# scroll-tech/zkevm-circuits

Measured on AMD Instinct MI355X. Metric: SuperCircuit-shape proof-gen wall-clock (s) at k = 20, lower is better.
Workload: dtype u32x8 limbs (254-bit modular integer, Montgomery)

## Files before the change

### zkevm-circuits_amd/csrc/ntt.hip

```cpp
#include "ctx.hpp"
#include "ff29.hip.hpp"

namespace zk {

constexpr int NTT_MAX_DIGIT = 10;
constexpr int NTT_TILE = 4096;
constexpr int NTT_THREADS = 1024;
constexpr int NTT_LDS_BYTES_PER_ELT = 36;

struct Tw29;

constexpr int NTT_BATCH = 16;
struct NttIo { const Fr* src[NTT_BATCH]; Fr* dst[NTT_BATCH]; };

struct NttPass {
    int log_np;
    int log_m;
    const Tw29* tw;
    const Fr* out_tw = nullptr;
};

struct NttDomain {
    uint32_t log_n = 0;
    int npass = 0;
    NttPass pass[3];
    int h = 0;
    Fr* d_lo = nullptr;
    Fr* d_hi = nullptr;
    Fr* d_tw[3] = {nullptr, nullptr, nullptr};
    Tw29* d_tw29[3] = {nullptr, nullptr, nullptr};
    Fr* d_out_tw[2] = {nullptr, nullptr};
    Fr final_mul;
    bool fin_folded = false;
    ~NttDomain() {
        if (d_lo) (void)hipFree(d_lo);
        if (d_hi) (void)hipFree(d_hi);
        for (auto p : d_tw) if (p) (void)hipFree(p);
        for (auto p : d_tw29) if (p) (void)hipFree((void*)p);
        for (auto p : d_out_tw) if (p) (void)hipFree(p);
    }
};

__device__ __forceinline__ uint32_t bitrev(uint32_t x, int bits) { return bits ? (__brev(x) >> (32 - bits)) : 0u; }

__host__ __device__ __forceinline__ Fr to_rprime(Fr x) {
#pragma unroll
    for (int i = 0; i < 5; ++i) x = dbl(x);
    return x;
}

struct Lds29 {
    uint32_t* p;
    int stride;
    __device__ __forceinline__ Fr29 load(int idx) const {
        Fr29 r;
#pragma unroll
        for (int k = 0; k < 9; ++k) r.l[k] = p[k * stride + idx];
        return r;
    }
    __device__ __forceinline__ void store(int idx, const Fr29& v) const {
#pragma unroll
        for (int k = 0; k < 9; ++k) p[k * stride + idx] = v.l[k];
    }
};

__global__ void k_powers(Fr base, Fr mul, Fr* out, uint32_t count, int rprime) {
    uint32_t j = blockIdx.x * blockDim.x + threadIdx.x;
    if (j >= count) return;
    Fr r = mul, b = base;
    uint32_t e = j;
    while (e) {
        if (e & 1) r = r * b;
        b = sqr(b);
        e >>= 1;
    }
    stg(out + j, rprime ? to_rprime(r) : r);
}

__device__ __forceinline__ Fr two_level(const Fr* __restrict__ lo, const Fr* __restrict__ hi, int h, uint32_t e) {
    return ldg(lo + (e & ((1u << h) - 1))) * ldg(hi + (e >> h));
}
__device__ __forceinline__ Fr29 two_level29(const Fr* __restrict__ lo, const Fr* __restrict__ hi, int h, uint32_t e) {
    return mul29(unpack29<Fr29P>(ldg(lo + (e & ((1u << h) - 1)))), unpack29<Fr29P>(ldg(hi + (e >> h))));
}

__global__ void k_build_out_twiddles(Fr* __restrict__ out_tw, const Fr* __restrict__ lo, const Fr* __restrict__ hi, int h, int log_np, int log_m, int tw_shift, uint64_t n,
                                     Fr fin, int apply_fin) {
    const uint64_t g = (uint64_t)blockIdx.x * blockDim.x + threadIdx.x;
    if (g >= n) return;
    const uint64_t m = 1ull << log_m;
    const uint32_t jpp = (uint32_t)(g & (m - 1)), d = (uint32_t)(g >> log_m) & ((1u << log_np) - 1);
    Fr29 v = two_level29(lo, hi, h, (jpp * d) << tw_shift);
    if (apply_fin) v = mul29(v, unpack29<Fr29P>(fin));
    stg(out_tw + g, pack29_lt2p(v));
}

__device__ __forceinline__ void bfly29(Fr29& u, Fr29& x, const Fr29& w) {
    const Fr29 v = mul29(x, w);
    Fr29 a0 = add29(u, v), a1 = sub29k<4>(u, v);
    normalize29(a0);
    normalize29(a1);
    u = a0;
    x = a1;
}
struct Tw29 { uint4 q[3]; };
__device__ __forceinline__ Fr29 tw29(const Tw29* __restrict__ tw, uint32_t idx) {
    const uint4 a = tw[idx].q[0], b = tw[idx].q[1], c = tw[idx].q[2];
    return Fr29{{a.x, a.y, a.z, a.w, b.x, b.y, b.z, b.w, c.x}};
}
__global__ void k_split_twiddles(const Fr* __restrict__ in, Tw29* __restrict__ out, uint32_t count) {
    const uint32_t i = blockIdx.x * blockDim.x + threadIdx.x;
    if (i >= count) return;
    const Fr29 v = unpack29<Fr29P>(ldg(in + i));
    out[i].q[0] = make_uint4(v.l[0], v.l[1], v.l[2], v.l[3]);
    out[i].q[1] = make_uint4(v.l[4], v.l[5], v.l[6], v.l[7]);
    out[i].q[2] = make_uint4(v.l[8], 0u, 0u, 0u);
}
__device__ __forceinline__ void bfly29_lazy(Fr29& u, Fr29& x, const Fr29& w) {
    const Fr29 v = mul29(x, w);
    const Fr29 a0 = add29(u, v), a1 = sub29k<2>(u, v);
    u = a0;
    x = a1;
}
template <int R>
__device__ __forceinline__ void dit_step(Fr29 (&e)[4], const Tw29* __restrict__ tw, int log_np, int s, int j) {
    const Fr29 w0 = tw29(tw, (uint32_t)j << (log_np - 1 - s));
    bfly29_lazy(e[0], e[1], w0);
    if (R == 2) {
        bfly29_lazy(e[2], e[3], w0);
        bfly29_lazy(e[0], e[2], tw29(tw, (uint32_t)j << (log_np - 2 - s)));
        bfly29_lazy(e[1], e[3], tw29(tw, (uint32_t)(j + (1 << s)) << (log_np - 2 - s)));
        normalize29(e[2]);
        normalize29(e[3]);
    }
    normalize29(e[0]);
    normalize29(e[1]);
}
__device__ __forceinline__ void bfly29_one(Fr29& u, Fr29& x) {
    Fr29 a0 = add29(u, x), a1 = sub29k<4>(u, x);
    normalize29(a0);
    normalize29(a1);
    u = a0;
    x = a1;
}
template <int R>
__device__ __forceinline__ void dit_first_step(Fr29 (&e)[4], const Tw29* __restrict__ tw, int log_np) {
    bfly29_one(e[0], e[1]);
    if (R == 2) {
        bfly29_one(e[2], e[3]);
        bfly29_one(e[0], e[2]);
        bfly29(e[1], e[3], tw29(tw, 1u << (log_np - 2)));
    }
}

__global__ void __launch_bounds__(NTT_THREADS)
k_ntt_pass(NttIo io, const Tw29* __restrict__ tw, const Fr* __restrict__ lo,
           const Fr* __restrict__ hi, int h, int log_np, int log_t, int log_m, int tw_shift, const Fr* __restrict__ pre,
           const Fr* __restrict__ out_tw, uint32_t ncols, int xcd_cols) {
    extern __shared__ __attribute__((aligned(16))) uint32_t smem[];
    uint32_t tile_id, col;
    if (xcd_cols) { const uint32_t slot = blockIdx.x >> 3; col = slot % ncols; tile_id = (slot / ncols) * 8u + (blockIdx.x & 7u); }
    else { col = blockIdx.x % ncols; tile_id = blockIdx.x / ncols; }
    const Fr* __restrict__ src = io.src[col];
    Fr* __restrict__ dst = io.dst[col];
    const int tile = 1 << (log_np + log_t);
    Lds29 L{smem, tile};
    const int T = 1 << log_t;
    const uint64_t m = 1ull << log_m;
    const uint32_t tiles_per_hi = (uint32_t)(m >> log_t);
    const uint32_t hi_idx = tile_id / tiles_per_hi, blk = tile_id % tiles_per_hi;
    const uint64_t base = ((uint64_t)hi_idx << (log_np + log_m)) + ((uint64_t)blk << log_t);

    for (int s = 0; s < log_np;) {
        const int r = ((log_np - s) & 1) ? 1 : 2;
        const bool first = s == 0, last = s + r == log_np;
        const int hgt = 1 << s, items = tile >> r;
        for (int it = threadIdx.x; it < items; it += blockDim.x) {
            const int c = it & (T - 1), b = it >> log_t;
            const int j = b & (hgt - 1);
            const int lo_d = ((b >> s) << (s + r)) | j;
            Fr29 e[4];
#pragma unroll
            for (int k = 0; k < 4; ++k) {
                if (k >= (1 << r)) break;
                const int dl = lo_d + k * hgt;
                if (first) {
                    const uint64_t gi = base + (uint64_t)bitrev(dl, log_np) * m + c;
                    e[k] = unpack29<Fr29P>(ldg(src + gi));
                    if (pre) e[k] = mul29(e[k], unpack29<Fr29P>(ldg(pre + gi)));
                } else {
                    e[k] = L.load((dl << log_t) | c);
                }
            }
            if (first) { if (r == 2) dit_first_step<2>(e, tw, log_np); else dit_first_step<1>(e, tw, log_np); }
            else if (r == 2) dit_step<2>(e, tw, log_np, s, j);
            else dit_step<1>(e, tw, log_np, s, j);
#pragma unroll
            for (int k = 0; k < 4; ++k) {
                if (k >= (1 << r)) break;
                const int dl = lo_d + k * hgt;
                if (last) {
                    const uint32_t jpp = (blk << log_t) + c;
                    const uint64_t go = base + (uint64_t)dl * m + c;
                    const Fr29 v = mul29(e[k], out_tw ? unpack29<Fr29P>(ldg(out_tw + go)) : two_level29(lo, hi, h, (jpp * (uint32_t)dl) << tw_shift));
                    stg(dst + go, pack29_raw(v));
                } else {
                    L.store((dl << log_t) | c, e[k]);
                }
            }
        }
        s += r;
        if (s < log_np) __syncthreads();
    }
}

static bool ntt_xcd_remap() { static const bool on = getenv("ZK_NTT_XCD") && atoi(getenv("ZK_NTT_XCD")) == 1; return on; }
__host__ __device__ __forceinline__ int ntt_row_pad(int log_np) { return log_np >= 8 ? 8 : 0; }
__global__ void __launch_bounds__(NTT_THREADS)
k_ntt_last(NttIo io, const Tw29* __restrict__ tw, int log_np, int log_t,
           int log_n1, int log_mid, Fr fin, const Fr* __restrict__ pre, int fin_folded, int xcd_remap) {
    extern __shared__ __attribute__((aligned(16))) uint32_t smem[];
    const Fr* __restrict__ src = io.src[blockIdx.y];
    Fr* __restrict__ dst = io.dst[blockIdx.y];
    const int tile = 1 << (log_np + log_t);
    const int T = 1 << log_t;
    const int row = (1 << log_np) + ntt_row_pad(log_np);
    Lds29 L{smem, T * row};
    uint32_t bx = blockIdx.x;
    if (xcd_remap) bx = (bx & 7u) * (gridDim.x >> 3) + (bx >> 3);
    const uint32_t mid = bx & ((1u << log_mid) - 1), blk = bx >> log_mid;
    const Fr29 fin29 = unpack29<Fr29P>(fin);

    for (int s = 0; s < log_np;) {
        const int r = ((log_np - s) & 1) ? 1 : 2;
        const bool first = s == 0, last = s + r == log_np;
        const int hgt = 1 << s, items = tile >> r;
        for (int it = threadIdx.x; it < items; it += blockDim.x) {
            int c, b;
            if (last) { c = it & (T - 1); b = it >> log_t; }
            else { b = it & ((1 << (log_np - r)) - 1); c = it >> (log_np - r); }
            const int j = b & (hgt - 1);
            const int lo_d = ((b >> s) << (s + r)) | j;
            const uint64_t i1 = ((uint64_t)blk << log_t) + c;
            Fr29 e[4];
#pragma unroll
            for (int k = 0; k < 4; ++k) {
                if (k >= (1 << r)) break;
                const int dl = lo_d + k * hgt;
                if (first) {
                    const uint64_t gi = (((i1 << log_mid) + mid) << log_np) + bitrev(dl, log_np);
                    e[k] = unpack29<Fr29P>(ldg(src + gi));
                    if (pre) e[k] = mul29(e[k], unpack29<Fr29P>(ldg(pre + gi)));
                } else {
                    e[k] = L.load(c * row + dl);
                }
            }
            if (first) { if (r == 2) dit_first_step<2>(e, tw, log_np); else dit_first_step<1>(e, tw, log_np); }
            else if (r == 2) dit_step<2>(e, tw, log_np, s, j);
            else dit_step<1>(e, tw, log_np, s, j);
#pragma unroll
            for (int k = 0; k < 4; ++k) {
                if (k >= (1 << r)) break;
                const int dl = lo_d + k * hgt;
                if (last) {
                    const uint64_t o = i1 + (((uint64_t)mid + ((uint64_t)dl << log_mid)) << log_n1);
                    stg(dst + o, fin_folded ? reduce_lazy29(e[k]) : pack29_lt2p(mul29(e[k], fin29)));
                } else {
                    L.store(c * row + dl, e[k]);
                }
            }
        }
        s += r;
        if (s < log_np) __syncthreads();
    }
}


template <int LOG_NP, int S, bool HAS_PRE>
__device__ __forceinline__ void ntt_pass_steps(const Lds29& L, const Fr* __restrict__ src, Fr* __restrict__ dst, const Tw29* __restrict__ tw,
                                               const Fr* __restrict__ pre, const Fr* __restrict__ out_tw, const int log_t, const uint64_t m, const uint64_t base) {
    constexpr int R = ((LOG_NP - S) & 1) ? 1 : 2, NE = 1 << R, hgt = 1 << S;
    constexpr bool FIRST = S == 0, LAST = S + R == LOG_NP;
    const int T = 1 << log_t, items = (1 << (LOG_NP + log_t)) >> R;
    for (int it = threadIdx.x; it < items; it += blockDim.x) {
        const int c = it & (T - 1), b = it >> log_t;
        const int j = b & (hgt - 1);
        const int lo_d = ((b >> S) << (S + R)) | j;
        Fr otw[NE];
        if (LAST) {
#pragma unroll
            for (int k = 0; k < NE; ++k) otw[k] = ldg(out_tw + base + (uint64_t)(lo_d + k * hgt) * m + c);
        }
        Fr29 e[4];
        if (FIRST) {
            Fr raw[NE], praw[NE];
#pragma unroll
            for (int k = 0; k < NE; ++k) {
                const uint64_t gi = base + (uint64_t)bitrev(lo_d + k * hgt, LOG_NP) * m + c;
                raw[k] = ldg(src + gi);
                if (HAS_PRE) praw[k] = ldg(pre + gi);
            }
#pragma unroll
            for (int k = 0; k < NE; ++k) {
                e[k] = unpack29<Fr29P>(raw[k]);
                if (HAS_PRE) e[k] = mul29(e[k], unpack29<Fr29P>(praw[k]));
            }
            dit_first_step<R>(e, tw, LOG_NP);
        } else {
#pragma unroll
            for (int k = 0; k < NE; ++k) e[k] = L.load(((lo_d + k * hgt) << log_t) | c);
            dit_step<R>(e, tw, LOG_NP, S, j);
        }
#pragma unroll
        for (int k = 0; k < NE; ++k) {
            const int dl = lo_d + k * hgt;
            if (LAST) stg(dst + base + (uint64_t)dl * m + c, pack29_raw(mul29(e[k], unpack29<Fr29P>(otw[k]))));
            else L.store((dl << log_t) | c, e[k]);
        }
    }
    if constexpr (!LAST) {
        __syncthreads();
        ntt_pass_steps<LOG_NP, S + R, HAS_PRE>(L, src, dst, tw, pre, out_tw, log_t, m, base);
    }
}
template <int LOG_NP, bool HAS_PRE>
__global__ void __launch_bounds__(NTT_THREADS)
k_ntt_pass_f(NttIo io, const Tw29* __restrict__ tw, int log_t, int log_m, const Fr* __restrict__ pre, const Fr* __restrict__ out_tw, uint32_t ncols, int xcd_cols, int log_grp) {
    extern __shared__ __attribute__((aligned(16))) uint32_t smem[];
    uint32_t tile_id, col;
    if (xcd_cols) {
        const uint32_t slot = blockIdx.x >> 3, sub = slot & ((1u << log_grp) - 1u), s2 = slot >> log_grp;
        col = s2 % ncols;
        tile_id = ((((s2 / ncols) << 3) + (blockIdx.x & 7u)) << log_grp) + sub;
    } else { col = blockIdx.x % ncols; tile_id = blockIdx.x / ncols; }
    Lds29 L{smem, 1 << (LOG_NP + log_t)};
    const uint64_t m = 1ull << log_m;
    const uint32_t tiles_per_hi = (uint32_t)(m >> log_t);
    const uint32_t hi_idx = tile_id / tiles_per_hi, blk = tile_id % tiles_per_hi;
    const uint64_t base = ((uint64_t)hi_idx << (LOG_NP + log_m)) + ((uint64_t)blk << log_t);
    ntt_pass_steps<LOG_NP, 0, HAS_PRE>(L, io.src[col], io.dst[col], tw, pre, out_tw, log_t, m, base);
}

template <int LOG_NP, int S>
__device__ __forceinline__ void ntt_last_steps(const Lds29& L, const Fr* __restrict__ src, Fr* __restrict__ dst, const Tw29* __restrict__ tw,
                                               const int log_t, const int row, const uint32_t blk, const uint32_t mid, const int log_mid, const int log_n1) {
    constexpr int R = ((LOG_NP - S) & 1) ? 1 : 2, NE = 1 << R, hgt = 1 << S;
    constexpr bool FIRST = S == 0, LAST = S + R == LOG_NP;
    const int T = 1 << log_t, items = (1 << (LOG_NP + log_t)) >> R;
    for (int it = threadIdx.x; it < items; it += blockDim.x) {
        int c, b;
        if (LAST) { c = it & (T - 1); b = it >> log_t; }
        else { b = it & ((1 << (LOG_NP - R)) - 1); c = it >> (LOG_NP - R); }
        const int j = b & (hgt - 1);
        const int lo_d = ((b >> S) << (S + R)) | j;
        const uint64_t i1 = ((uint64_t)blk << log_t) + c;
        Fr29 e[4];
        if (FIRST) {
            Fr raw[NE];
#pragma unroll
            for (int k = 0; k < NE; ++k) raw[k] = ldg(src + ((((i1 << log_mid) + mid) << LOG_NP) + bitrev(lo_d + k * hgt, LOG_NP)));
#pragma unroll
            for (int k = 0; k < NE; ++k) e[k] = unpack29<Fr29P>(raw[k]);
            dit_first_step<R>(e, tw, LOG_NP);
        } else {
#pragma unroll
            for (int k = 0; k < NE; ++k) e[k] = L.load(c * row + lo_d + k * hgt);
            dit_step<R>(e, tw, LOG_NP, S, j);
        }
#pragma unroll
        for (int k = 0; k < NE; ++k) {
            const int dl = lo_d + k * hgt;
            if (LAST) stg(dst + (i1 + (((uint64_t)mid + ((uint64_t)dl << log_mid)) << log_n1)), reduce_lazy29(e[k]));
            else L.store(c * row + dl, e[k]);
        }
    }
    if constexpr (!LAST) {
        __syncthreads();
        ntt_last_steps<LOG_NP, S + R>(L, src, dst, tw, log_t, row, blk, mid, log_mid, log_n1);
    }
}
template <int LOG_NP>
__global__ void __launch_bounds__(NTT_THREADS)
k_ntt_last_f(NttIo io, const Tw29* __restrict__ tw, int log_t, int log_n1, int log_mid, int xcd_remap) {
    extern __shared__ __attribute__((aligned(16))) uint32_t smem[];
    const int row = (1 << LOG_NP) + ntt_row_pad(LOG_NP);
    Lds29 L{smem, (1 << log_t) * row};
    uint32_t bx = blockIdx.x;
    if (xcd_remap) bx = (bx & 7u) * (gridDim.x >> 3) + (bx >> 3);
    const uint32_t mid = bx & ((1u << log_mid) - 1), blk = bx >> log_mid;
    ntt_last_steps<LOG_NP, 0>(L, io.src[blockIdx.y], io.dst[blockIdx.y], tw, log_t, row, blk, mid, log_mid, log_n1);
}

__global__ void k_scale(Fr* a, Fr s, uint64_t n) {
    uint64_t i = (uint64_t)blockIdx.x * blockDim.x + threadIdx.x;
    if (i < n) stg(a + i, ldg(a + i) * s);
}
int fr_scale_run(zk_ctx* ctx, Fr* d_a, const Fr& s, uint64_t n) {
    if (!n) return ZK_OK;
    hipLaunchKernelGGL(k_scale, dim3((unsigned)((n + 255) / 256)), dim3(256), 0, ctx->stream, d_a, s, n);
    ZK_CHECK_LAUNCH(ctx);
    return ZK_OK;
}

__global__ void k_distribute_powers(const Fr* src, Fr* dst, const Fr* __restrict__ lo, const Fr* __restrict__ hi, int h, uint64_t n) {
    uint64_t i = (uint64_t)blockIdx.x * blockDim.x + threadIdx.x;
    if (i >= n) return;
    stg(dst + i, ldg(src + i) * two_level(lo, hi, h, (uint32_t)i));
}

static int build_powers(zk_ctx* ctx, const Fr& base, const Fr& mul, Fr* d_out, uint32_t count, int rprime) {
    hipLaunchKernelGGL(k_powers, dim3((count + 255) / 256), dim3(256), 0, ctx->stream, base, mul, d_out, count, rprime);
    ZK_CHECK_LAUNCH(ctx);
    return ZK_OK;
}

static uint64_t domain_key(uint32_t log_n, const Fr& omega, const Fr* scale) {
    uint64_t hsh = 1469598103934665603ull;
    auto mix = [&](uint32_t v) { hsh = (hsh ^ v) * 1099511628211ull; };
    mix(log_n);
    for (int i = 0; i < 8; ++i) mix(omega.l[i]);
    if (scale) for (int i = 0; i < 8; ++i) mix(scale->l[i] ^ 0x9e3779b9u);
    return hsh;
}

static int get_domain(zk_ctx* ctx, uint32_t log_n, const Fr& omega, const Fr* scale, std::shared_ptr<NttDomain>* out) {
    const uint64_t key = domain_key(log_n, omega, scale);
    auto it = ctx->domains.find(key);
    if (it != ctx->domains.end()) { *out = it->second; return ZK_OK; }
    auto d = std::make_shared<NttDomain>();
    d->log_n = log_n;
    d->final_mul = to_rprime(scale ? *scale : Fr::one());
    const int P = log_n <= NTT_MAX_DIGIT ? 1 : (log_n <= 2 * NTT_MAX_DIGIT ? 2 : 3);
    d->npass = P;
    int rem = (int)log_n;
    for (int p = 0; p < P; ++p) {
        int b = (rem + (P - p) - 1) / (P - p);
        d->pass[p].log_np = b;
        rem -= b;
        d->pass[p].log_m = rem;
    }
    if (P > 1) {
        d->h = (int)(log_n + 1) / 2;
        const uint32_t nlo = 1u << d->h, nhi = 1u << (log_n - d->h);
        ZK_HIP(ctx, hipMalloc(&d->d_lo, sizeof(Fr) * nlo));
        ZK_HIP(ctx, hipMalloc(&d->d_hi, sizeof(Fr) * nhi));
        int rc = build_powers(ctx, omega, Fr::one(), d->d_lo, nlo, 1);
        if (rc) return rc;
        Fr step = omega;
        for (int i = 0; i < d->h; ++i) step = sqr(step);
        rc = build_powers(ctx, step, Fr::one(), d->d_hi, nhi, 1);
        if (rc) return rc;
    }
    for (int p = 0; p < P; ++p) {
        const int b = d->pass[p].log_np;
        const uint32_t cnt = b ? (1u << (b - 1)) : 1u;
        ZK_HIP(ctx, hipMalloc(&d->d_tw[p], sizeof(Fr) * cnt));
        Fr w = omega;
        for (uint32_t i = 0; i < log_n - (uint32_t)b; ++i) w = sqr(w);
        int rc = build_powers(ctx, w, Fr::one(), d->d_tw[p], cnt, 1);
        if (rc) return rc;
        ZK_HIP(ctx, hipMalloc((void**)&d->d_tw29[p], sizeof(Tw29) * cnt));
        hipLaunchKernelGGL(k_split_twiddles, dim3((cnt + 255) / 256), dim3(256), 0, ctx->stream, (const Fr*)d->d_tw[p], d->d_tw29[p], cnt);
        ZK_CHECK_LAUNCH(ctx);
        d->pass[p].tw = d->d_tw29[p];
    }
    if (P > 1 && log_n <= 24) {
        const uint64_t n = 1ull << log_n;
        for (int p = 0; p + 1 < P; ++p) {
            if (hipMalloc(&d->d_out_tw[p], sizeof(Fr) * n) != hipSuccess) { (void)hipGetLastError(); d->d_out_tw[p] = nullptr; break; }
            const NttPass& ps = d->pass[p];
            hipLaunchKernelGGL(k_build_out_twiddles, dim3((unsigned)((n + 255) / 256)), dim3(256), 0, ctx->stream, d->d_out_tw[p], (const Fr*)d->d_lo, (const Fr*)d->d_hi, d->h,
                               ps.log_np, ps.log_m, (int)log_n - ps.log_np - ps.log_m, n, d->final_mul, p == P - 2 ? 1 : 0);
            ZK_CHECK_LAUNCH(ctx);
            d->pass[p].out_tw = d->d_out_tw[p];
            if (p == P - 2) d->fin_folded = true;
        }
    }
    if (ctx->domains.size() > 64) ctx->domains.clear();
    ctx->domains[key] = d;
    *out = d;
    return ZK_OK;
}

static int set_lds_attr(zk_ctx* ctx) {
    if (ctx->ntt_attr_set) return ZK_OK;
    ZK_HIP(ctx, hipFuncSetAttribute((const void*)k_ntt_pass, hipFuncAttributeMaxDynamicSharedMemorySize, NTT_TILE * NTT_LDS_BYTES_PER_ELT));
    ZK_HIP(ctx, hipFuncSetAttribute((const void*)k_ntt_last, hipFuncAttributeMaxDynamicSharedMemorySize, (NTT_TILE + 128) * NTT_LDS_BYTES_PER_ELT));
    ctx->ntt_attr_set = true;
    return ZK_OK;
}


template <int LOG_NP, bool HAS_PRE>
static bool launch_pass_f(zk_ctx* ctx, unsigned grid, unsigned threads, size_t lds, const NttIo& io, const Tw29* tw, int log_t, int log_m, const Fr* pre, const Fr* out_tw, uint32_t ncols, int xcd_cols, int log_grp) {
    const uint32_t bit = 1u << (2 * (LOG_NP - 7) + (HAS_PRE ? 1 : 0));
    if (!(ctx->ntt_fixed_attr & bit)) {
        if (hipFuncSetAttribute((const void*)k_ntt_pass_f<LOG_NP, HAS_PRE>, hipFuncAttributeMaxDynamicSharedMemorySize, NTT_TILE * NTT_LDS_BYTES_PER_ELT) != hipSuccess) { (void)hipGetLastError(); return false; }
        ctx->ntt_fixed_attr |= bit;
    }
    hipLaunchKernelGGL((k_ntt_pass_f<LOG_NP, HAS_PRE>), dim3(grid), dim3(threads), lds, ctx->stream, io, tw, log_t, log_m, pre, out_tw, ncols, xcd_cols, log_grp);
    return true;
}
static bool ntt_fixed_on() { const char* e = getenv("ZK_NTT_FIXED"); return !(e && atoi(e) == 0); }
static bool launch_pass_fixed(zk_ctx* ctx, int log_np, unsigned grid, unsigned threads, size_t lds, const NttIo& io, const Tw29* tw, int log_t, int log_m, const Fr* pre, const Fr* out_tw, uint32_t ncols, int xcd_cols, int log_grp) {
    if (!ntt_fixed_on() || !out_tw) return false;
#define ZK_PASS_CASE(N) case N: return pre ? launch_pass_f<N, true>(ctx, grid, threads, lds, io, tw, log_t, log_m, pre, out_tw, ncols, xcd_cols, log_grp) \
                                           : launch_pass_f<N, false>(ctx, grid, threads, lds, io, tw, log_t, log_m, pre, out_tw, ncols, xcd_cols, log_grp);
    switch (log_np) { ZK_PASS_CASE(7) ZK_PASS_CASE(8) ZK_PASS_CASE(9) ZK_PASS_CASE(10) ZK_PASS_CASE(11) default: return false; }
#undef ZK_PASS_CASE
}
template <int LOG_NP>
static bool launch_last_f(zk_ctx* ctx, dim3 grid, unsigned threads, size_t lds, const NttIo& io, const Tw29* tw, int log_t, int log_n1, int log_mid, int xcd_remap) {
    const uint32_t bit = 1u << (24 + LOG_NP - 7);
    if (!(ctx->ntt_fixed_attr & bit)) {
        if (hipFuncSetAttribute((const void*)k_ntt_last_f<LOG_NP>, hipFuncAttributeMaxDynamicSharedMemorySize, (NTT_TILE + 128) * NTT_LDS_BYTES_PER_ELT) != hipSuccess) { (void)hipGetLastError(); return false; }
        ctx->ntt_fixed_attr |= bit;
    }
    hipLaunchKernelGGL((k_ntt_last_f<LOG_NP>), grid, dim3(threads), lds, ctx->stream, io, tw, log_t, log_n1, log_mid, xcd_remap);
    return true;
}
static bool launch_last_fixed(zk_ctx* ctx, int log_np, dim3 grid, unsigned threads, size_t lds, const NttIo& io, const Tw29* tw, int log_t, int log_n1, int log_mid, int xcd_remap) {
    if (!ntt_fixed_on()) return false;
#define ZK_LAST_CASE(N) case N: return launch_last_f<N>(ctx, grid, threads, lds, io, tw, log_t, log_n1, log_mid, xcd_remap);
    switch (log_np) { ZK_LAST_CASE(7) ZK_LAST_CASE(8) ZK_LAST_CASE(9) ZK_LAST_CASE(10) ZK_LAST_CASE(11) default: return false; }
#undef ZK_LAST_CASE
}

static int pick_threads(int tile) { return tile >= 4096 ? 1024 : (tile >= 1024 ? 512 : (tile >= 256 ? 128 : 64)); }

int ntt_run_many(zk_ctx* ctx, Fr* const* d_datas, const Fr* const* d_srcs, size_t count, uint32_t log_n, const Fr& omega, const Fr* scale, const Fr* coset_pre, const Fr* coset_post, bool fuse_pre);
int ntt_run(zk_ctx* ctx, Fr* d_data, uint32_t log_n, const Fr& omega, const Fr* scale, const Fr* coset_pre, const Fr* coset_post, const Fr* d_src, bool fuse_pre) {
    return ntt_run_many(ctx, &d_data, d_src ? &d_src : nullptr, 1, log_n, omega, scale, coset_pre, coset_post, fuse_pre);
}
int ntt_run_many(zk_ctx* ctx, Fr* const* d_datas, const Fr* const* d_srcs, size_t count, uint32_t log_n, const Fr& omega, const Fr* scale, const Fr* coset_pre, const Fr* coset_post, bool fuse_pre) {
    if (count == 0) return ZK_OK;
    if (count > 1 && (log_n == 0 || coset_post)) {
        for (size_t i = 0; i < count; ++i) {
            const Fr* one_src = d_srcs ? d_srcs[i] : nullptr;
            int r = ntt_run_many(ctx, d_datas + i, one_src ? &one_src : nullptr, 1, log_n, omega, scale, coset_pre, coset_post, fuse_pre);
            if (r) return r;
        }
        return ZK_OK;
    }
    Fr* d_data = d_datas[0];
    const Fr* d_src = d_srcs ? d_srcs[0] : nullptr;
    if (log_n == 0) {
        if (d_src && d_src != d_data) ZK_HIP(ctx, hipMemcpyAsync(d_data, d_src, sizeof(Fr), hipMemcpyDeviceToDevice, ctx->stream));
        if (scale) {
            hipLaunchKernelGGL(k_scale, dim3(1), dim3(64), 0, ctx->stream, d_data, *scale, (uint64_t)1);
            ZK_CHECK_LAUNCH(ctx);
        }
        return ZK_OK;
    }
    int rc = set_lds_attr(ctx);
    if (rc) return rc;
    const uint64_t n = 1ull << log_n;

    auto run_distribute = [&](const Fr& g, const Fr* from) -> int {
        const int h = (int)(log_n + 1) / 2;
        const uint32_t nlo = 1u << h, nhi = 1u << (log_n - h);
        const uint64_t key = domain_key(log_n, g, nullptr) ^ 0xC05E7ull;
        Fr* tab = nullptr;
        auto it = ctx->pow_tables.find(key);
        if (it != ctx->pow_tables.end()) {
            tab = (Fr*)it->second;
        } else {
            if (hipMalloc(&tab, sizeof(Fr) * ((size_t)nlo + nhi)) != hipSuccess) return ctx->fail(ZK_ERR_OOM, "coset table allocation failed");
            int r = build_powers(ctx, g, Fr::one(), tab, nlo, 0);
            if (r) return r;
            Fr step = g;
            for (int i = 0; i < h; ++i) step = sqr(step);
            r = build_powers(ctx, step, Fr::one(), tab + nlo, nhi, 0);
            if (r) return r;
            ctx->pow_tables[key] = tab;
        }
        hipLaunchKernelGGL(k_distribute_powers, dim3((unsigned)((n + 255) / 256)), dim3(256), 0, ctx->stream, from, d_data, tab, tab + nlo, h, n);
        ZK_CHECK_LAUNCH(ctx);
        return ZK_OK;
    };
    const Fr* cur = d_src ? d_src : d_data;
    const Fr* pre_table = nullptr;
    if (coset_pre && fuse_pre) {
        const uint64_t key = domain_key(log_n, *coset_pre, nullptr) ^ 0xF0117ABull;
        auto it = ctx->pow_tables.find(key);
        if (it != ctx->pow_tables.end()) {
            pre_table = (const Fr*)it->second;
        } else {
            Fr* tab = nullptr;
            if (hipMalloc(&tab, sizeof(Fr) * n) != hipSuccess) { (void)hipGetLastError(); tab = nullptr; }
            if (tab) {
                int r = build_powers(ctx, *coset_pre, Fr::one(), tab, (uint32_t)n, 1);
                if (r) return r;
                ctx->pow_tables[key] = tab;
                pre_table = tab;
            }
        }
    }
    if (coset_pre && !pre_table) {
        if (count > 1) {
            for (size_t i = 0; i < count; ++i) {
                const Fr* one_src = d_srcs ? d_srcs[i] : nullptr;
                int r = ntt_run_many(ctx, d_datas + i, one_src ? &one_src : nullptr, 1, log_n, omega, scale, coset_pre, coset_post, fuse_pre);
                if (r) return r;
            }
            return ZK_OK;
        }
        rc = run_distribute(*coset_pre, cur); if (rc) return rc; cur = d_data;
    }

    std::shared_ptr<NttDomain> dom;
    rc = get_domain(ctx, log_n, omega, scale, &dom);
    if (rc) return rc;
    const int P = dom->npass;
    size_t per_launch = 1;
    if (count > 1) {
        const uint64_t tiles = std::max<uint64_t>(1, n >> 12);
        per_launch = (size_t)std::min<uint64_t>(NTT_BATCH, std::max<uint64_t>(1, 4096 / tiles));
        if (const char* e = getenv("ZK_NTT_BATCH")) { const int v = atoi(e); if (v >= 1 && v <= NTT_BATCH) per_launch = (size_t)v; }
    }
    Fr* scratch = nullptr;
    if (P > 1) {
        const int slot = ctx->stream_aux && ctx->stream == ctx->stream_aux ? SC_NTT_AUX : SC_NTT;
        for (;;) {
            scratch = (Fr*)ctx->get_scratch(slot, sizeof(Fr) * n * per_launch);
            if (scratch || per_launch == 1) break;
            (void)hipGetLastError();
            per_launch = (per_launch + 1) / 2;
        }
        if (!scratch) return ZK_ERR_OOM;
    }
    for (size_t first = 0; first < count; first += per_launch) {
        const size_t nb = std::min(per_launch, count - first);
        NttIo io_in{}, io_mid{}, io_last{};
        for (size_t j = 0; j < nb; ++j) {
            Fr* dd = d_datas[first + j];
            const Fr* ss = (count == 1) ? cur : (d_srcs && d_srcs[first + j] ? d_srcs[first + j] : dd);
            io_in.src[j] = ss;
            io_in.dst[j] = dd;
        }
        NttIo cur_io = io_in;
        for (int p = 0; p + 1 < P; ++p) {
            const NttPass& ps = dom->pass[p];
            int log_tile_pass = P == 3 ? 11 : 12;
            if (const char* e = getenv("ZK_NTT_PASS_LOGTILE")) { const int v = atoi(e); if (v >= 10 && v <= 12) log_tile_pass = v; }
            int log_t = log_tile_pass - ps.log_np;
            if (log_t < 0) log_t = 0;
            if (log_t > ps.log_m) log_t = ps.log_m;
            const int tile = 1 << (ps.log_np + log_t);
            NttIo io{};
            for (size_t j = 0; j < nb; ++j) {
                io.src[j] = cur_io.src[j];
                io.dst[j] = (p == P - 2) ? scratch + j * n : d_datas[first + j];
            }
            const unsigned blocks = (unsigned)(n >> (ps.log_np + log_t));
            const int tw_shift = (int)log_n - ps.log_np - ps.log_m;
            ZkProfScope pscope(ctx, "ntt_pass");
            pscope.bytes = (uint64_t)nb * n * 64 / (uint64_t)P;
            static const bool xcd_off = getenv("ZK_NTT_XCD_COLS") && atoi(getenv("ZK_NTT_XCD_COLS")) == 0;
            const int xcd_cols = (nb > 1 && blocks % 8 == 0 && !xcd_off) ? 1 : 0;
            const int log_grp = log_t < 2 ? 2 - log_t : 0;
            const int xcd_fixed = (!xcd_off && blocks % (8u << log_grp) == 0 && (nb > 1 || log_grp > 0)) ? 1 : 0;
            if (!launch_pass_fixed(ctx, ps.log_np, blocks * (unsigned)nb, (unsigned)std::max(64, std::min(1024, tile >> 2)) , (size_t)tile * NTT_LDS_BYTES_PER_ELT, io, ps.tw, log_t, ps.log_m,
                                   p == 0 ? pre_table : (const Fr*)nullptr, ps.out_tw, (uint32_t)nb, xcd_fixed, xcd_fixed ? log_grp : 0))
                hipLaunchKernelGGL(k_ntt_pass, dim3(blocks * (unsigned)nb), dim3(pick_threads(tile)), (size_t)tile * NTT_LDS_BYTES_PER_ELT, ctx->stream, io, ps.tw,
                                   dom->d_lo, dom->d_hi, dom->h, ps.log_np, log_t, ps.log_m, tw_shift, p == 0 ? pre_table : (const Fr*)nullptr, ps.out_tw,
                                   (uint32_t)nb, xcd_cols);
            ZK_CHECK_LAUNCH(ctx);
            for (size_t j = 0; j < nb; ++j) cur_io.src[j] = io.dst[j];
        }
        {
            const NttPass& ps = dom->pass[P - 1];
            const int log_n1 = P == 1 ? 0 : dom->pass[0].log_np;
            const int log_mid = P == 3 ? dom->pass[1].log_np : 0;
            int log_tile_last = 11;
            if (const char* e = getenv("ZK_NTT_LAST_LOGTILE")) { const int v = atoi(e); if (v >= 10 && v <= 12) log_tile_last = v; }
            int log_t = log_tile_last - ps.log_np;
            if (log_t < 0) log_t = 0;
            if (log_t > log_n1) log_t = log_n1;
            const int tile = 1 << (ps.log_np + log_t);
            const unsigned blocks = (unsigned)(n >> (ps.log_np + log_t));
            NttIo io{};
            for (size_t j = 0; j < nb; ++j) { io.src[j] = cur_io.src[j]; io.dst[j] = d_datas[first + j]; }
            ZkProfScope pscope(ctx, "ntt_last");
            pscope.bytes = (uint64_t)nb * n * 64 / (uint64_t)P;
            const int xcd_last = (log_mid == 0 && blocks % 8 == 0 && blocks >= 16 && ntt_xcd_remap()) ? 1 : 0;
            const size_t lds_last = (size_t)(tile + (ntt_row_pad(ps.log_np) << log_t)) * NTT_LDS_BYTES_PER_ELT;
            if (!(P > 1 && dom->fin_folded && launch_last_fixed(ctx, ps.log_np, dim3(blocks, (unsigned)nb), (unsigned)std::max(64, std::min(1024, tile >> 2)), lds_last, io, ps.tw, log_t, log_n1, log_mid, xcd_last)))
                hipLaunchKernelGGL(k_ntt_last, dim3(blocks, (unsigned)nb), dim3(pick_threads(tile)), lds_last, ctx->stream, io, ps.tw,
                                   ps.log_np, log_t, log_n1, log_mid, dom->final_mul, P == 1 ? pre_table : (const Fr*)nullptr, dom->fin_folded ? 1 : 0, xcd_last);
            ZK_CHECK_LAUNCH(ctx);
        }
    }
    if (coset_post) { rc = run_distribute(*coset_post, d_data); if (rc) return rc; }
    return ZK_OK;
}

template <int W>
__global__ void __launch_bounds__(256) k_ntt_cross(const Fr* __restrict__ recv, Fr* __restrict__ out, size_t cols, const Fr* __restrict__ tw , Fr scale, int scaled) {
    const size_t c = (size_t)blockIdx.x * blockDim.x + threadIdx.x;
    if (c >= cols) return;
    constexpr int LOGW = W == 2 ? 1 : W == 4 ? 2 : W == 8 ? 3 : 4;
    Fr a[W];
#pragma unroll
    for (int i = 0; i < W; ++i) {
        int rev = 0;
#pragma unroll
        for (int b = 0; b < LOGW; ++b) rev |= ((i >> b) & 1) << (LOGW - 1 - b);
        a[rev] = ldg(recv + (size_t)i * cols + c);
    }
#pragma unroll
    for (int st = 1; st <= LOGW; ++st) {
#pragma unroll
        for (int h = 0; h < W / 2; ++h) {
            const int half = 1 << (st - 1), t = h & (half - 1), lo = ((h >> (st - 1)) << st) + t, hi = lo + half;
            const Fr u = a[lo];
            const Fr v = t == 0 ? a[hi] : a[hi] * tw[t << (LOGW - st)];
            a[lo] = u + v;
            a[hi] = u - v;
        }
    }
#pragma unroll
    for (int j = 0; j < W; ++j) stg(out + (size_t)j * cols + c, scaled ? a[j] * scale : a[j]);
}

}

using namespace zk;
extern "C" int zk_ntt_sharded(zk_ctx* ctx, void* d_local, uint32_t log_n, int inverse, uint32_t rank, uint32_t world, zk_alltoall_fn exchange, void* user) {
    if (!ctx) return ZK_ERR_INVALID_ARG;
    ZK_REQUIRE(ctx, d_local, "null pointer");
    ZK_REQUIRE(ctx, exchange || world == 1 || (comm_ready(ctx) && ctx->comm_world == world && ctx->comm_rank == rank), "no all-to-all callback and no matching communicator (zk_comm_init)");
    ZK_REQUIRE(ctx, world >= 1 && world <= 16 && (world & (world - 1)) == 0 && rank < world, "world must be a power of two <= 16, rank < world");
    ZK_REQUIRE(ctx, log_n <= 28, "log_n exceeds the two-adicity of Fr (28)");
    uint32_t log_w = 0;
    while ((1u << log_w) < world) ++log_w;
    ZK_REQUIRE(ctx, log_n >= 2 * log_w, "need n >= world^2");
    if (world == 1) return zk_ntt(ctx, d_local, log_n, inverse);
    const uint32_t log_m = log_n - log_w;
    const size_t m = (size_t)1 << log_m, cols = m >> log_w;
    Fr w_n = fr_root_of_unity(log_n), w_m = fr_root_of_unity(log_m), w_w = fr_root_of_unity(log_w);
    if (inverse) { w_n = fr_inv_host(w_n); w_m = fr_inv_host(w_m); w_w = fr_inv_host(w_w); }
    const Fr g = fr_pow(w_n, rank);
    int rc = ntt_run(ctx, (Fr*)d_local, log_m, w_m, nullptr, nullptr, rank ? &g : nullptr);
    if (rc) return rc;
    Fr* recv = (Fr*)ctx->pool_get(m * sizeof(Fr));
    Fr* d_tw = (Fr*)ctx->pool_get(16 * sizeof(Fr));
    if (!recv || !d_tw) { ctx->pool_put(recv, m * sizeof(Fr)); ctx->pool_put(d_tw, 16 * sizeof(Fr)); return ctx->fail(ZK_ERR_OOM, "sharded NTT: exchange buffer of %zu bytes", m * sizeof(Fr)); }
    auto done = [&](int code) { ctx->pool_put(recv, m * sizeof(Fr)); ctx->pool_put(d_tw, 16 * sizeof(Fr)); return code; };
    hipError_t e = hipSuccess;
    if (exchange) {
        e = hipStreamSynchronize(ctx->stream);
        if (e != hipSuccess) return done(ctx->fail(ZK_ERR_HIP, "sharded NTT: %s", hipGetErrorString(e)));
        if (exchange(user, d_local, cols * sizeof(Fr), recv) != 0) return done(ctx->fail(ZK_ERR_INVALID_ARG, "sharded NTT: the all-to-all callback failed"));
    } else {
        rc = comm_alltoall_dev(ctx, d_local, cols * sizeof(Fr), recv);
        if (rc) return done(rc);
    }
    Fr tw[8];
    tw[0] = Fr::one();
    for (uint32_t t = 1; t < (world > 1 ? world / 2 : 1); ++t) tw[t] = tw[t - 1] * w_w;
    e = hipMemcpyAsync(d_tw, tw, sizeof(Fr) * (world / 2 ? world / 2 : 1), hipMemcpyHostToDevice, ctx->stream);
    if (e != hipSuccess) return done(ctx->fail(ZK_ERR_HIP, "sharded NTT: %s", hipGetErrorString(e)));
    const Fr ninv = inverse ? fr_inv_host(fr_from_u64(1ull << log_n)) : Fr::one();
    const dim3 grid((unsigned)((cols + 255) / 256)), block(256);
    switch (world) {
        case 2: hipLaunchKernelGGL(k_ntt_cross<2>, grid, block, 0, ctx->stream, (const Fr*)recv, (Fr*)d_local, cols, (const Fr*)d_tw, ninv, inverse); break;
        case 4: hipLaunchKernelGGL(k_ntt_cross<4>, grid, block, 0, ctx->stream, (const Fr*)recv, (Fr*)d_local, cols, (const Fr*)d_tw, ninv, inverse); break;
        case 8: hipLaunchKernelGGL(k_ntt_cross<8>, grid, block, 0, ctx->stream, (const Fr*)recv, (Fr*)d_local, cols, (const Fr*)d_tw, ninv, inverse); break;
        default: hipLaunchKernelGGL(k_ntt_cross<16>, grid, block, 0, ctx->stream, (const Fr*)recv, (Fr*)d_local, cols, (const Fr*)d_tw, ninv, inverse); break;
    }
    e = hipGetLastError();
    if (e != hipSuccess) return done(ctx->fail(ZK_ERR_HIP, "sharded NTT: %s", hipGetErrorString(e)));
    e = hipStreamSynchronize(ctx->stream);
    if (e != hipSuccess) return done(ctx->fail(ZK_ERR_HIP, "sharded NTT: %s", hipGetErrorString(e)));
    return done(ZK_OK);
}
```

Before: 1.876.

## Remap NTT butterfly work so most steps need only wavefront barriers

Adds a wave-level work mapping for the fixed-radix NTT pass and last-pass kernels. Each 64-lane wavefront owns a closed set of 256 elements across consecutive butterfly steps, so block-wide __syncthreads is replaced by a wavefront fence plus wave barrier everywhere except at one split step. This targets the cost of repeated workgroup barriers in 1024-thread blocks, at the price of extra index arithmetic and possibly worse LDS bank or global coalescing patterns. It is enabled by default and can be disabled with an environment variable.

```diff
diff --git a/zkevm-circuits_amd/csrc/ntt.hip b/zkevm-circuits_amd/csrc/ntt.hip
--- a/zkevm-circuits_amd/csrc/ntt.hip
+++ b/zkevm-circuits_amd/csrc/ntt.hip
@@ -1,5 +1,6 @@
 #include "ctx.hpp"
 #include "ff29.hip.hpp"
+#include "ntt_wave_map.hpp"
 
 namespace zk {
 
@@ -276,16 +277,19 @@
 }
 
 
-template <int LOG_NP, int S, bool HAS_PRE>
+__device__ __forceinline__ void ntt_wave_sync() {
+    __builtin_amdgcn_fence(__ATOMIC_RELEASE, "wavefront");
+    __builtin_amdgcn_wave_barrier();
+    __builtin_amdgcn_fence(__ATOMIC_ACQUIRE, "wavefront");
+}
+template <int LOG_NP, int S, bool HAS_PRE, bool WAVE>
 __device__ __forceinline__ void ntt_pass_steps(const Lds29& L, const Fr* __restrict__ src, Fr* __restrict__ dst, const Tw29* __restrict__ tw,
-                                               const Fr* __restrict__ pre, const Fr* __restrict__ out_tw, const int log_t, const uint64_t m, const uint64_t base) {
+                                               const Fr* __restrict__ pre, const Fr* __restrict__ out_tw, const int log_t, const uint64_t m, const uint64_t base, const NttWaveMap& wm) {
     constexpr int R = ((LOG_NP - S) & 1) ? 1 : 2, NE = 1 << R, hgt = 1 << S;
     constexpr bool FIRST = S == 0, LAST = S + R == LOG_NP;
     const int T = 1 << log_t, items = (1 << (LOG_NP + log_t)) >> R;
-    for (int it = threadIdx.x; it < items; it += blockDim.x) {
-        const int c = it & (T - 1), b = it >> log_t;
-        const int j = b & (hgt - 1);
-        const int lo_d = ((b >> S) << (S + R)) | j;
+    auto item = [&](const int c, const int lo_d) __attribute__((always_inline)) {
+        const int j = lo_d & (hgt - 1);
         Fr otw[NE];
         if (LAST) {
 #pragma unroll
@@ -317,13 +321,26 @@
             if (LAST) stg(dst + base + (uint64_t)dl * m + c, pack29_raw(mul29(e[k], unpack29<Fr29P>(otw[k]))));
             else L.store((dl << log_t) | c, e[k]);
         }
+    };
+    if constexpr (WAVE) {
+        const int nsets = 1 << (LOG_NP + log_t - wm.wb), per = 1 << (wm.wb - R);
+        for (int w = threadIdx.x >> 6; w < nsets; w += blockDim.x >> 6)
+            for (int li = threadIdx.x & 63; li < per; li += 64) {
+                const NttWaveItem wi = ntt_wave_item(wm, LOG_NP, log_t, false, S, R, w, li);
+                item(wi.c, wi.lo_d);
+            }
+    } else {
+        for (int it = threadIdx.x; it < items; it += blockDim.x) {
+            const int c = it & (T - 1), b = it >> log_t;
+            item(c, ((b >> S) << (S + R)) | (b & (hgt - 1)));
+        }
     }
     if constexpr (!LAST) {
-        __syncthreads();
-        ntt_pass_steps<LOG_NP, S + R, HAS_PRE>(L, src, dst, tw, pre, out_tw, log_t, m, base);
-    }
-}
-template <int LOG_NP, bool HAS_PRE>
+        if constexpr (WAVE && S + R != ntt_wave_split(LOG_NP, false)) ntt_wave_sync(); else __syncthreads();
+        ntt_pass_steps<LOG_NP, S + R, HAS_PRE, WAVE>(L, src, dst, tw, pre, out_tw, log_t, m, base, wm);
+    }
+}
+template <int LOG_NP, bool HAS_PRE, bool WAVE>
 __global__ void __launch_bounds__(NTT_THREADS)
 k_ntt_pass_f(NttIo io, const Tw29* __restrict__ tw, int log_t, int log_m, const Fr* __restrict__ pre, const Fr* __restrict__ out_tw, uint32_t ncols, int xcd_cols, int log_grp) {
     extern __shared__ __attribute__((aligned(16))) uint32_t smem[];
@@ -338,21 +355,18 @@
     const uint32_t tiles_per_hi = (uint32_t)(m >> log_t);
     const uint32_t hi_idx = tile_id / tiles_per_hi, blk = tile_id % tiles_per_hi;
     const uint64_t base = ((uint64_t)hi_idx << (LOG_NP + log_m)) + ((uint64_t)blk << log_t);
-    ntt_pass_steps<LOG_NP, 0, HAS_PRE>(L, io.src[col], io.dst[col], tw, pre, out_tw, log_t, m, base);
-}
-
-template <int LOG_NP, int S>
+    const NttWaveMap wm = ntt_wave_map(LOG_NP, log_t, false);
+    ntt_pass_steps<LOG_NP, 0, HAS_PRE, WAVE>(L, io.src[col], io.dst[col], tw, pre, out_tw, log_t, m, base, wm);
+}
+
+template <int LOG_NP, int S, bool WAVE>
 __device__ __forceinline__ void ntt_last_steps(const Lds29& L, const Fr* __restrict__ src, Fr* __restrict__ dst, const Tw29* __restrict__ tw,
-                                               const int log_t, const int row, const uint32_t blk, const uint32_t mid, const int log_mid, const int log_n1) {
+                                               const int log_t, const int row, const uint32_t blk, const uint32_t mid, const int log_mid, const int log_n1, const NttWaveMap& wm) {
     constexpr int R = ((LOG_NP - S) & 1) ? 1 : 2, NE = 1 << R, hgt = 1 << S;
     constexpr bool FIRST = S == 0, LAST = S + R == LOG_NP;
     const int T = 1 << log_t, items = (1 << (LOG_NP + log_t)) >> R;
-    for (int it = threadIdx.x; it < items; it += blockDim.x) {
-        int c, b;
-        if (LAST) { c = it & (T - 1); b = it >> log_t; }
-        else { b = it & ((1 << (LOG_NP - R)) - 1); c = it >> (LOG_NP - R); }
-        const int j = b & (hgt - 1);
-        const int lo_d = ((b >> S) << (S + R)) | j;
+    auto item = [&](const int c, const int lo_d) __attribute__((always_inline)) {
+        const int j = lo_d & (hgt - 1);
         const uint64_t i1 = ((uint64_t)blk << log_t) + c;
         Fr29 e[4];
         if (FIRST) {
@@ -373,13 +387,28 @@
             if (LAST) stg(dst + (i1 + (((uint64_t)mid + ((uint64_t)dl << log_mid)) << log_n1)), reduce_lazy29(e[k]));
             else L.store(c * row + dl, e[k]);
         }
+    };
+    if constexpr (WAVE) {
+        const int nsets = 1 << (LOG_NP + log_t - wm.wb), per = 1 << (wm.wb - R);
+        for (int w = threadIdx.x >> 6; w < nsets; w += blockDim.x >> 6)
+            for (int li = threadIdx.x & 63; li < per; li += 64) {
+                const NttWaveItem wi = ntt_wave_item(wm, LOG_NP, log_t, !LAST, S, R, w, li);
+                item(wi.c, wi.lo_d);
+            }
+    } else {
+        for (int it = threadIdx.x; it < items; it += blockDim.x) {
+            int c, b;
+            if (LAST) { c = it & (T - 1); b = it >> log_t; }
+            else { b = it & ((1 << (LOG_NP - R)) - 1); c = it >> (LOG_NP - R); }
+            item(c, ((b >> S) << (S + R)) | (b & (hgt - 1)));
+        }
     }
     if constexpr (!LAST) {
-        __syncthreads();
-        ntt_last_steps<LOG_NP, S + R>(L, src, dst, tw, log_t, row, blk, mid, log_mid, log_n1);
-    }
-}
-template <int LOG_NP>
+        if constexpr (WAVE && S + R != ntt_wave_split(LOG_NP, true)) ntt_wave_sync(); else __syncthreads();
+        ntt_last_steps<LOG_NP, S + R, WAVE>(L, src, dst, tw, log_t, row, blk, mid, log_mid, log_n1, wm);
+    }
+}
+template <int LOG_NP, bool WAVE>
 __global__ void __launch_bounds__(NTT_THREADS)
 k_ntt_last_f(NttIo io, const Tw29* __restrict__ tw, int log_t, int log_n1, int log_mid, int xcd_remap) {
     extern __shared__ __attribute__((aligned(16))) uint32_t smem[];
@@ -388,7 +417,8 @@
     uint32_t bx = blockIdx.x;
     if (xcd_remap) bx = (bx & 7u) * (gridDim.x >> 3) + (bx >> 3);
     const uint32_t mid = bx & ((1u << log_mid) - 1), blk = bx >> log_mid;
-    ntt_last_steps<LOG_NP, 0>(L, io.src[blockIdx.y], io.dst[blockIdx.y], tw, log_t, row, blk, mid, log_mid, log_n1);
+    const NttWaveMap wm = ntt_wave_map(LOG_NP, log_t, true);
+    ntt_last_steps<LOG_NP, 0, WAVE>(L, io.src[blockIdx.y], io.dst[blockIdx.y], tw, log_t, row, blk, mid, log_mid, log_n1, wm);
 }
 
 __global__ void k_scale(Fr* a, Fr s, uint64_t n) {
@@ -491,17 +521,22 @@
 }
 
 
+static bool ntt_fixed_on() { const char* e = getenv("ZK_NTT_FIXED"); return !(e && atoi(e) == 0); }
+static bool ntt_wave_on() { const char* e = getenv("ZK_NTT_WAVE"); return !(e && atoi(e) == 0); }
 template <int LOG_NP, bool HAS_PRE>
 static bool launch_pass_f(zk_ctx* ctx, unsigned grid, unsigned threads, size_t lds, const NttIo& io, const Tw29* tw, int log_t, int log_m, const Fr* pre, const Fr* out_tw, uint32_t ncols, int xcd_cols, int log_grp) {
     const uint32_t bit = 1u << (2 * (LOG_NP - 7) + (HAS_PRE ? 1 : 0));
     if (!(ctx->ntt_fixed_attr & bit)) {
-        if (hipFuncSetAttribute((const void*)k_ntt_pass_f<LOG_NP, HAS_PRE>, hipFuncAttributeMaxDynamicSharedMemorySize, NTT_TILE * NTT_LDS_BYTES_PER_ELT) != hipSuccess) { (void)hipGetLastError(); return false; }
+        if (hipFuncSetAttribute((const void*)k_ntt_pass_f<LOG_NP, HAS_PRE, false>, hipFuncAttributeMaxDynamicSharedMemorySize, NTT_TILE * NTT_LDS_BYTES_PER_ELT) != hipSuccess ||
+            hipFuncSetAttribute((const void*)k_ntt_pass_f<LOG_NP, HAS_PRE, true>, hipFuncAttributeMaxDynamicSharedMemorySize, NTT_TILE * NTT_LDS_BYTES_PER_ELT) != hipSuccess) { (void)hipGetLastError(); return false; }
         ctx->ntt_fixed_attr |= bit;
     }
-    hipLaunchKernelGGL((k_ntt_pass_f<LOG_NP, HAS_PRE>), dim3(grid), dim3(threads), lds, ctx->stream, io, tw, log_t, log_m, pre, out_tw, ncols, xcd_cols, log_grp);
+    if (ntt_wave_on() && threads % 64 == 0 && ntt_wave_map(LOG_NP, log_t, false).valid)
+        hipLaunchKernelGGL((k_ntt_pass_f<LOG_NP, HAS_PRE, true>), dim3(grid), dim3(threads), lds, ctx->stream, io, tw, log_t, log_m, pre, out_tw, ncols, xcd_cols, log_grp);
+    else
+        hipLaunchKernelGGL((k_ntt_pass_f<LOG_NP, HAS_PRE, false>), dim3(grid), dim3(threads), lds, ctx->stream, io, tw, log_t, log_m, pre, out_tw, ncols, xcd_cols, log_grp);
     return true;
 }
-static bool ntt_fixed_on() { const char* e = getenv("ZK_NTT_FIXED"); return !(e && atoi(e) == 0); }
 static bool launch_pass_fixed(zk_ctx* ctx, int log_np, unsigned grid, unsigned threads, size_t lds, const NttIo& io, const Tw29* tw, int log_t, int log_m, const Fr* pre, const Fr* out_tw, uint32_t ncols, int xcd_cols, int log_grp) {
     if (!ntt_fixed_on() || !out_tw) return false;
 #define ZK_PASS_CASE(N) case N: return pre ? launch_pass_f<N, true>(ctx, grid, threads, lds, io, tw, log_t, log_m, pre, out_tw, ncols, xcd_cols, log_grp) \
@@ -513,10 +548,14 @@
 static bool launch_last_f(zk_ctx* ctx, dim3 grid, unsigned threads, size_t lds, const NttIo& io, const Tw29* tw, int log_t, int log_n1, int log_mid, int xcd_remap) {
     const uint32_t bit = 1u << (24 + LOG_NP - 7);
     if (!(ctx->ntt_fixed_attr & bit)) {
-        if (hipFuncSetAttribute((const void*)k_ntt_last_f<LOG_NP>, hipFuncAttributeMaxDynamicSharedMemorySize, (NTT_TILE + 128) * NTT_LDS_BYTES_PER_ELT) != hipSuccess) { (void)hipGetLastError(); return false; }
+        if (hipFuncSetAttribute((const void*)k_ntt_last_f<LOG_NP, false>, hipFuncAttributeMaxDynamicSharedMemorySize, (NTT_TILE + 128) * NTT_LDS_BYTES_PER_ELT) != hipSuccess ||
+            hipFuncSetAttribute((const void*)k_ntt_last_f<LOG_NP, true>, hipFuncAttributeMaxDynamicSharedMemorySize, (NTT_TILE + 128) * NTT_LDS_BYTES_PER_ELT) != hipSuccess) { (void)hipGetLastError(); return false; }
         ctx->ntt_fixed_attr |= bit;
     }
-    hipLaunchKernelGGL((k_ntt_last_f<LOG_NP>), grid, dim3(threads), lds, ctx->stream, io, tw, log_t, log_n1, log_mid, xcd_remap);
+    if (ntt_wave_on() && threads % 64 == 0 && ntt_wave_map(LOG_NP, log_t, true).valid)
+        hipLaunchKernelGGL((k_ntt_last_f<LOG_NP, true>), grid, dim3(threads), lds, ctx->stream, io, tw, log_t, log_n1, log_mid, xcd_remap);
+    else
+        hipLaunchKernelGGL((k_ntt_last_f<LOG_NP, false>), grid, dim3(threads), lds, ctx->stream, io, tw, log_t, log_n1, log_mid, xcd_remap);
     return true;
 }
 static bool launch_last_fixed(zk_ctx* ctx, int log_np, dim3 grid, unsigned threads, size_t lds, const NttIo& io, const Tw29* tw, int log_t, int log_n1, int log_mid, int xcd_remap) {
diff --git a/zkevm-circuits_amd/csrc/ntt_wave_map.hpp b/zkevm-circuits_amd/csrc/ntt_wave_map.hpp
--- /dev/null
+++ b/zkevm-circuits_amd/csrc/ntt_wave_map.hpp
@@ -0,0 +1,73 @@
+#pragma once
+
+#if defined(__HIPCC__) || defined(__CUDACC__)
+#define ZK_WM_HD __host__ __device__ inline __attribute__((always_inline))
+#else
+#define ZK_WM_HD inline
+#endif
+
+namespace zk {
+
+constexpr int NTT_WAVE_LOG_ELTS = 8;
+
+constexpr int ntt_step_radix(int log_np, int s) { return ((log_np - s) & 1) ? 1 : 2; }
+
+constexpr int ntt_wave_split(int log_np, bool last_pass) {
+    const int amax = last_pass ? NTT_WAVE_LOG_ELTS : NTT_WAVE_LOG_ELTS - 2;
+    int sa = 0;
+    for (int s = 0; s < log_np; s += ntt_step_radix(log_np, s))
+        if (s > 0 && s <= amax && log_np - s <= NTT_WAVE_LOG_ELTS - 2) sa = s;
+    return sa;
+}
+
+struct NttWaveMap {
+    int valid;
+    int wb;
+    int sa;
+    int a_nc, a_d;
+    int b_nc, b_p;
+};
+
+ZK_WM_HD NttWaveMap ntt_wave_map(int log_np, int log_t, bool last_pass) {
+    NttWaveMap m{};
+    const int e = log_np + log_t;
+    m.wb = e < NTT_WAVE_LOG_ELTS ? e : NTT_WAVE_LOG_ELTS;
+    m.sa = ntt_wave_split(log_np, last_pass);
+    const int hb = log_np - m.sa, cmin = log_t < 2 ? log_t : 2;
+    if (m.sa == 0 || m.sa > m.wb || hb > m.wb) return m;
+    if (last_pass) { m.a_d = log_np < m.wb ? log_np : m.wb; m.a_nc = m.wb - m.a_d; }
+    else { m.a_nc = log_t < m.wb - m.sa ? log_t : m.wb - m.sa; m.a_d = m.wb - m.a_nc; }
+    m.b_nc = log_t < m.wb - hb ? log_t : m.wb - hb;
+    m.b_p = m.wb - hb - m.b_nc;
+    m.valid = m.sa <= m.a_d && (last_pass || m.a_nc >= cmin) && m.b_nc >= cmin;
+    return m;
+}
+
+ZK_WM_HD int ntt_wave_barriers(const NttWaveMap& m, int log_np) {
+    if (m.valid) return 1;
+    int steps = 0;
+    for (int s = 0; s < log_np; s += ntt_step_radix(log_np, s)) ++steps;
+    return steps - 1;
+}
+
+struct NttWaveItem { int c, lo_d; };
+ZK_WM_HD NttWaveItem ntt_wave_item(const NttWaveMap& m, int log_np, int log_t, bool d_fastest, int s, int r, int set, int li) {
+    NttWaveItem it;
+    if (s < m.sa) {
+        const int c_hi = set & ((1 << (log_t - m.a_nc)) - 1), d_hi = set >> (log_t - m.a_nc);
+        int c_lo, b;
+        if (d_fastest) { b = li & ((1 << (m.a_d - r)) - 1); c_lo = li >> (m.a_d - r); }
+        else { c_lo = li & ((1 << m.a_nc) - 1); b = li >> m.a_nc; }
+        it.c = (c_hi << m.a_nc) | c_lo;
+        it.lo_d = (d_hi << m.a_d) | ((b >> s) << (s + r)) | (b & ((1 << s) - 1));
+    } else {
+        const int c_hi = set & ((1 << (log_t - m.b_nc)) - 1), d_mid = set >> (log_t - m.b_nc);
+        const int c_lo = li & ((1 << m.b_nc) - 1), rest = li >> m.b_nc;
+        const int p = rest & ((1 << m.b_p) - 1), hb = rest >> m.b_p, sh = s - m.sa;
+        it.c = (c_hi << m.b_nc) | c_lo;
+        it.lo_d = ((((hb >> sh) << (sh + r)) | (hb & ((1 << sh) - 1))) << m.sa) | (d_mid << m.b_p) | p;
+    }
+    return it;
+}
+
+}
```

Result: no change. 1.862 (median of 6 runs) (-0.8%).
